# pmgbergen/porepy

Measured on AMD Instinct MI355X. Metric: cells/sec MPFA assemble+solve, 3D unstructured grid, higher is better.
Workload: dtype f64

## Files before the change

include/porefv.h:

```cpp
#ifndef POREFV_H
#define POREFV_H

#include <stddef.h>
#include <stdint.h>

#ifdef __cplusplus
extern "C" {
#endif

typedef struct pfv_ctx pfv_ctx;

typedef enum {
  PFV_OK = 0,
  PFV_ERR_SINGULAR = 1,
  PFV_ERR_CELL_SHAPE = 2,
  PFV_ERR_HIP = 3,
  PFV_ERR_ARGUMENT = 4,
  PFV_ERR_UNSUPPORTED = 5,
  PFV_ERR_NOT_CONVERGED = 6
} pfv_status;

enum {
  PFV_MAT_FLUX = 0,
  PFV_MAT_BOUND_FLUX = 1,
// ... 25 lines not shown
       PFV_PRECOND_AMG_NNS = 3,
       PFV_PRECOND_SWEEP = 4     };

enum {
  PFV_FLUXFN_LINEAR = 0,
  PFV_FLUXFN_COREY = 1,
  PFV_FLUXFN_TABLE = 2
};

enum {
  PFV_DISCR_REBUILD_TOPOLOGY = 1,
  PFV_DISCR_SKIP_VECTOR_SOURCE = 2
};

typedef struct {
  int32_t iterations;
  int32_t converged;
  double rel_residual;
  double solve_ms;
} pfv_solve_info;

typedef struct {
  double topology_ms;
  double symbolic_ms;
  double node_ms;
  double face_ms;
  double assemble_ms;
  double solve_ms;
  double bytes_written_outputs;
  int64_t num_nodes, num_sub_half_faces, sum_block_sq, max_block;
  double amg_setup_ms;
  double amg_operator_complexity;
  int64_t amg_levels, amg_coarsest_rows;
  double discretize_ms;
  int64_t solve_renumbered;
  double node_flops;
  int64_t node_table_doubles;
  int64_t amg_maps_reused;
  int64_t amg_level0_nnz;
  double amg_filter_theta;
  int64_t win_reused;
  int64_t amg_filter_layout;
  int64_t solve_launches;
  int64_t amg_setup_launches;
  int64_t node_redo;
  int64_t symbolic_reused;
  int64_t amg_stale_rematches;
  int64_t mpsa_contrast_regions;
  double mpsa_max_contrast;
  int64_t assemble_positions_kept;
  int64_t pipeline_runs;
  int64_t amg_nns_modes;
  double face_flux_ms;
  double upwind_ms;
  double transport_assemble_ms;
  double transport_advance_ms;
  int64_t transport_iterations;
  int64_t transport_gmres_retries;
  double advdiff_assemble_ms;
  double advdiff_advance_ms;
  int64_t advdiff_iterations;
  int64_t advdiff_precond_fallbacks;
  int64_t advdiff_gmres_retries;
  int64_t sweep_levels;
  int64_t sweep_core_cells;
  int64_t sweep_launches;
  double sweep_order_ms;
  int64_t sweep_direct_steps;
  int64_t sweep_direct_fallbacks;
  int64_t transport_multi_components;
  int64_t transport_multi_direct_steps;
  int64_t transport_multi_fallback_components;
  double transport_nl_ms;
  int64_t transport_nl_steps;
  int64_t transport_nl_core_iterations;
  int64_t transport_nl_components;
  double transport_react_ms;
  int64_t transport_react_steps;
  int64_t transport_react_core_iterations;
  int64_t transport_react_components;
  double transport_adjoint_ms;
  int64_t transport_adjoint_steps;
  int64_t transport_adjoint_core_iterations;
} pfv_stats;

pfv_status pfv_create(int device, pfv_ctx** out);
void pfv_destroy(pfv_ctx* h);
const char* pfv_last_error(pfv_ctx* h);
int pfv_is_device_build(void);

pfv_status pfv_set_grid(pfv_ctx* h, int nd, int64_t nc, int64_t nf, int64_t nn,
                        const double* nodes, const int32_t* cf_indptr,
                        const int32_t* cf_indices, const int8_t* cf_sign,
                        const int32_t* fn_indptr, const int32_t* fn_indices,
                        const double* face_normals, const double* face_centers,
                        const double* cell_centers, const double* face_areas);

pfv_status pfv_mpfa_set_params(pfv_ctx* h, const double* perm_33n, const uint8_t* bc_flags,
                               const double* robin_weight, double eta,
                               const double* eta_subface);

pfv_status pfv_mpfa_set_permeability(pfv_ctx* h, const double* perm_33n);

#define PFV_AD_WANT_FLUX_JACOBIAN 1u
pfv_status pfv_mpfa_ad_flux_system(pfv_ctx* h, const double* p, const double* dk_dp, const double* bc_values,
                                   const double* vector_source, const double* source, double* flux_out,
                                   uint32_t flags);

pfv_status pfv_mpfa_set_subface_bc(pfv_ctx* h, const uint8_t* bc_flags_sub, const double* robin_weight_sub);

pfv_status pfv_mpfa_discretize(pfv_ctx* h, uint32_t flags);

pfv_status pfv_tpfa_discretize(pfv_ctx* h, int vector_source_dim);

pfv_status pfv_tpfa_transmissibility_ad(pfv_ctx* h, const double* perm_33n, double* t_face, double* dt_dk);

pfv_status pfv_mpfa_discretize_faces(pfv_ctx* h, uint32_t flags, int64_t n_faces,
                                     const int32_t* faces, int keep_other_rows);

pfv_status pfv_matrix_info(pfv_ctx* h, int which, int64_t* nrows, int64_t* ncols,
                           int64_t* nnz);
pfv_status pfv_get_matrix(pfv_ctx* h, int which, int32_t* indptr, int32_t* indices,
                          double* data);
pfv_status pfv_device_memory(pfv_ctx* h, int64_t* free_bytes, int64_t* total_bytes);
pfv_status pfv_host_alloc(size_t bytes, void** out);
void pfv_host_free(void* p);
pfv_status pfv_active_size(pfv_ctx* h, int64_t* n);
pfv_status pfv_get_matrix_rows(pfv_ctx* h, int which, int64_t n_rows, const int32_t* rows, int32_t* out_indptr,
                               int32_t* out_indices, double* out_data);

pfv_status pfv_mpfa_assemble(pfv_ctx* h, const double* bc_values, const double* vector_source,
                             const double* source);
pfv_status pfv_get_rhs(pfv_ctx* h, double* b);

pfv_status pfv_spmv(pfv_ctx* h, int which, const double* x, double* y);

enum {
  PFV_BIOT_SCALAR_GRADIENT = 0,
  PFV_BIOT_DISPLACEMENT_DIVERGENCE = 1,
  PFV_BIOT_BOUNDARY_DISPLACEMENT_DIVERGENCE = 2,
  PFV_BIOT_CONSISTENCY = 3,
  PFV_BIOT_BOUND_DISPLACEMENT_PRESSURE = 4,
  PFV_BIOT_NUM_TERMS = 5
};
pfv_status pfv_biot_set_alphas(pfv_ctx* h, int nalpha, const double* alpha_k33n);
pfv_status pfv_biot_discretize_faces(pfv_ctx* h, uint32_t flags, int64_t n_faces, const int32_t* faces,
                                     int64_t n_cells, const int32_t* cells, int keep_other_rows);

pfv_status pfv_biot_discretize(pfv_ctx* h, uint32_t flags);
pfv_status pfv_biot_matrix_info(pfv_ctx* h, int term, int64_t* nrows, int64_t* ncols, int64_t* nnz);
pfv_status pfv_biot_get_matrix(pfv_ctx* h, int term, int key, int32_t* indptr, int32_t* indices,
                               double* data);

pfv_status pfv_set_system(pfv_ctx* h, int64_t n, const int32_t* indptr, const int32_t* indices,
                          const double* data, const double* rhs);

pfv_status pfv_set_periodic(pfv_ctx* h, const int32_t* native_cell, const double* shift);

pfv_status pfv_set_vectors_on_device(pfv_ctx* h, int on);

pfv_status pfv_set_preconditioner(pfv_ctx* h, int kind);

pfv_status pfv_sweep_info(pfv_ctx* h, int64_t info[4], int32_t* level, int32_t* order);

pfv_status pfv_set_near_null_space(pfv_ctx* h, int bs, int k, const double* B);

// ... 144 lines not shown
```

porepy_amd/_lib.py:

```python
from __future__ import annotations

import ctypes as C
import os

import numpy as np

_HERE = os.path.dirname(os.path.abspath(__file__))
DEFAULT_LIBRARY = os.path.join(_HERE, "csrc", "libporefv_hip.so")

MAT_FLUX, MAT_BOUND_FLUX, MAT_BOUND_PRESSURE_CELL, MAT_BOUND_PRESSURE_FACE = 0, 1, 2, 3
MAT_VECTOR_SOURCE, MAT_BOUND_PRESSURE_VECTOR_SOURCE, MAT_SYSTEM = 4, 5, 6
MAT_STRESS, MAT_BOUND_STRESS, MAT_BOUND_DISPLACEMENT_CELL, MAT_BOUND_DISPLACEMENT_FACE, MAT_MECH_SYSTEM = 7, 8, 9, 10, 11
MAT_USER_SYSTEM = 12
MAT_FLUX_JACOBIAN = 13
MAT_UPWIND, MAT_UPWIND_RHS_DIR, MAT_UPWIND_RHS_NEU, MAT_TRANSPORT_SYSTEM = 14, 15, 16, 17
MAT_ADVDIFF_SYSTEM = 18
BC_DIR, BC_NEU, BC_ROB, BC_INTERNAL = 1, 2, 4, 8
SOLVE_CG, SOLVE_BICGSTAB, SOLVE_GMRES = 0, 1, 2
PRECOND_JACOBI, PRECOND_AMG, PRECOND_BLOCK, PRECOND_AMG_NNS, PRECOND_SWEEP = 0, 1, 2, 3, 4
FLUXFN_LINEAR, FLUXFN_COREY, FLUXFN_TABLE = 0, 1, 2
DISCR_REBUILD_TOPOLOGY, DISCR_SKIP_VECTOR_SOURCE = 1, 2

STATUS_NAMES = {
    0: "ok", 1: "singular local system", 2: "unsupported cell shape", 3: "HIP error",
    4: "bad argument", 5: "unsupported size/feature", 6: "not converged",
}

EXPORTS = [
    "pfv_create", "pfv_destroy", "pfv_last_error", "pfv_is_device_build", "pfv_set_grid",
    "pfv_mpfa_set_params", "pfv_mpfa_discretize", "pfv_matrix_info", "pfv_get_matrix",
    "pfv_mpfa_assemble", "pfv_get_rhs", "pfv_spmv", "pfv_solve", "pfv_spmv_device",
    "pfv_get_device_rhs", "pfv_sync", "pfv_get_stats", "pfv_time_kernel", "pfv_debug_copy",
    "pfv_spmv_device_rows", "pfv_copy_device_vector", "pfv_set_stream",
    "pfv_mpsa_set_params", "pfv_mpsa_discretize", "pfv_mpsa_assemble",
    "pfv_mpfa_discretize_faces", "pfv_set_system", "pfv_tpfa_discretize", "pfv_mpsa_discretize_faces", "pfv_set_preconditioner", "pfv_amg_setup", "pfv_amg_setup_sharded", "pfv_amg_apply_device", "pfv_csr_from_host", "pfv_csr_from_matrix", "pfv_csr_block_diag", "pfv_csr_matmul", "pfv_csr_axpby", "pfv_csr_transpose", "pfv_csr_bmat", "pfv_csr_scale", "pfv_csr_divide", "pfv_csr_spmv", "pfv_csr_spmv_device", "pfv_csr_info", "pfv_csr_get", "pfv_csr_set_system", "pfv_csr_free", "pfv_reset_stream", "pfv_mpsa_set_robin", "pfv_mpsa_set_basis", "pfv_mpfa_set_subface_bc", "pfv_mpsa_set_subface_bc", "pfv_mpsa_set_subface_basis",
    "pfv_biot_set_alphas", "pfv_biot_discretize", "pfv_biot_matrix_info", "pfv_biot_get_matrix",
    "pfv_set_vectors_on_device", "pfv_set_periodic", "pfv_biot_discretize_faces", "pfv_solve_sharded", "pfv_tpfa_transmissibility_ad",
    "pfv_get_matrix_rows", "pfv_active_size", "pfv_device_memory",
    "pfv_rccl_unique_id", "pfv_rccl_comm_create", "pfv_rccl_set_halo_plan", "pfv_rccl_hooks", "pfv_rccl_stats",
    "pfv_rccl_last_error", "pfv_rccl_comm_destroy", "pfv_mpfa_ad_flux_system", "pfv_host_alloc", "pfv_host_free",
    "pfv_mpsa_set_subface_eta", "pfv_mpsa_set_reconstruction_eta", "pfv_mpsa_set_reconstruction_eta_subface", "pfv_get_stats_n", "pfv_set_block_preconditioner",
    "pfv_mpfa_set_permeability", "pfv_set_near_null_space", "pfv_amg_nns_level", "pfv_amg_level",
    "pfv_mpfa_face_flux", "pfv_upwind_set_bc", "pfv_upwind_discretize", "pfv_upwind_assemble", "pfv_transport_advance",
    "pfv_advdiff_assemble", "pfv_advdiff_advance", "pfv_advdiff_face_flux", "pfv_resident_flux",
    "pfv_sweep_info", "pfv_transport_advance_multi", "pfv_transport_advance_nl", "pfv_transport_advance_nl_multi",
    "pfv_transport_advance_react", "pfv_transport_adjoint_multi",
]


class SolveInfo(C.Structure):
    _fields_ = [("iterations", C.c_int32), ("converged", C.c_int32),
                ("rel_residual", C.c_double), ("solve_ms", C.c_double)]


class Stats(C.Structure):
    _fields_ = [("topology_ms", C.c_double), ("symbolic_ms", C.c_double), ("node_ms", C.c_double),
                ("face_ms", C.c_double), ("assemble_ms", C.c_double), ("solve_ms", C.c_double),
                ("bytes_written_outputs", C.c_double), ("num_nodes", C.c_int64),
                ("num_sub_half_faces", C.c_int64), ("sum_block_sq", C.c_int64),
                ("max_block", C.c_int64), ("amg_setup_ms", C.c_double),
                ("amg_operator_complexity", C.c_double), ("amg_levels", C.c_int64),
                ("amg_coarsest_rows", C.c_int64), ("discretize_ms", C.c_double), ("solve_renumbered", C.c_int64),
                ("node_flops", C.c_double), ("node_table_doubles", C.c_int64),
                ("amg_maps_reused", C.c_int64), ("amg_level0_nnz", C.c_int64), ("amg_filter_theta", C.c_double),
                ("win_reused", C.c_int64), ("amg_filter_layout", C.c_int64),
                ("solve_launches", C.c_int64), ("amg_setup_launches", C.c_int64), ("node_redo", C.c_int64),
                ("symbolic_reused", C.c_int64), ("amg_stale_rematches", C.c_int64),
                ("mpsa_contrast_regions", C.c_int64), ("mpsa_max_contrast", C.c_double), ("assemble_positions_kept", C.c_int64),
                ("pipeline_runs", C.c_int64), ("amg_nns_modes", C.c_int64),
                ("face_flux_ms", C.c_double), ("upwind_ms", C.c_double), ("transport_assemble_ms", C.c_double),
                ("transport_advance_ms", C.c_double), ("transport_iterations", C.c_int64),
                ("transport_gmres_retries", C.c_int64),
                ("advdiff_assemble_ms", C.c_double), ("advdiff_advance_ms", C.c_double),
                ("advdiff_iterations", C.c_int64), ("advdiff_precond_fallbacks", C.c_int64),
                ("advdiff_gmres_retries", C.c_int64),
                ("sweep_levels", C.c_int64), ("sweep_core_cells", C.c_int64), ("sweep_launches", C.c_int64),
                ("sweep_order_ms", C.c_double), ("sweep_direct_steps", C.c_int64),
                ("sweep_direct_fallbacks", C.c_int64),
                ("transport_multi_components", C.c_int64), ("transport_multi_direct_steps", C.c_int64),
                ("transport_multi_fallback_components", C.c_int64),
                ("transport_nl_ms", C.c_double), ("transport_nl_steps", C.c_int64),
                ("transport_nl_core_iterations", C.c_int64), ("transport_nl_components", C.c_int64),
                ("transport_react_ms", C.c_double), ("transport_react_steps", C.c_int64),
                ("transport_react_core_iterations", C.c_int64), ("transport_react_components", C.c_int64),
                ("transport_adjoint_ms", C.c_double), ("transport_adjoint_steps", C.c_int64),
                ("transport_adjoint_core_iterations", C.c_int64)]

    def as_dict(self):
        return {n: getattr(self, n) for n, _ in self._fields_}


HALO_FN = C.CFUNCTYPE(C.c_int, C.c_void_p, C.c_void_p, C.c_void_p)
ALLREDUCE_FN = C.CFUNCTYPE(C.c_int, C.c_void_p, C.c_void_p, C.c_int, C.c_void_p)


SENDRECV_FN = C.CFUNCTYPE(C.c_int, C.c_void_p, C.c_int, C.POINTER(C.c_int32), C.c_void_p, C.POINTER(C.c_int64),
                          C.c_void_p, C.POINTER(C.c_int64), C.c_void_p)
ALLGATHER_FN = C.CFUNCTYPE(C.c_int, C.c_void_p, C.c_void_p, C.c_void_p, C.c_int64, C.c_void_p)


class ShardHooks(C.Structure):
    _fields_ = [("exchange_halo", HALO_FN), ("allreduce_sum", ALLREDUCE_FN), ("user", C.c_void_p),
                ("sendrecv", SENDRECV_FN), ("allgather", ALLGATHER_FN)]


class PorefvError(RuntimeError):
    def __init__(self, status: int, message: str):
        super().__init__(f"porefv status {status} ({STATUS_NAMES.get(status, '?')}): {message}")
        self.status = status
        self.message = message


_dp = C.POINTER(C.c_double)
_ip = C.POINTER(C.c_int32)
_bp = C.POINTER(C.c_int8)
_up = C.POINTER(C.c_uint8)
_lp = C.POINTER(C.c_int64)
_h = C.c_void_p


def _bind(lib: C.CDLL) -> C.CDLL:
    lib.pfv_create.argtypes = [C.c_int, C.POINTER(_h)]
    lib.pfv_create.restype = C.c_int
    lib.pfv_destroy.argtypes = [_h]
    lib.pfv_destroy.restype = None
    lib.pfv_last_error.argtypes = [_h]
    lib.pfv_last_error.restype = C.c_char_p
    lib.pfv_is_device_build.argtypes = []
    lib.pfv_is_device_build.restype = C.c_int
    lib.pfv_set_grid.argtypes = [_h, C.c_int, C.c_int64, C.c_int64, C.c_int64, _dp, _ip, _ip, _bp,
                                 _ip, _ip, _dp, _dp, _dp, _dp]
    lib.pfv_set_grid.restype = C.c_int
    lib.pfv_mpfa_set_params.argtypes = [_h, _dp, _up, _dp, C.c_double, _dp]
    lib.pfv_mpfa_set_params.restype = C.c_int
    lib.pfv_mpfa_set_permeability.argtypes = [_h, _dp]
    lib.pfv_mpfa_set_permeability.restype = C.c_int
    lib.pfv_mpfa_discretize.argtypes = [_h, C.c_uint32]
    lib.pfv_mpfa_discretize.restype = C.c_int
    lib.pfv_mpfa_discretize_faces.argtypes = [_h, C.c_uint32, C.c_int64, _ip, C.c_int]
    lib.pfv_mpfa_discretize_faces.restype = C.c_int
    lib.pfv_mpsa_discretize_faces.argtypes = [_h, C.c_uint32, C.c_int64, _ip, C.c_int]
    lib.pfv_mpsa_discretize_faces.restype = C.c_int
    lib.pfv_biot_set_alphas.argtypes = [_h, C.c_int, _dp]
    lib.pfv_biot_set_alphas.restype = C.c_int
    lib.pfv_biot_discretize.argtypes = [_h, C.c_uint32]
    lib.pfv_biot_discretize.restype = C.c_int
    lib.pfv_biot_matrix_info.argtypes = [_h, C.c_int, _lp, _lp, _lp]
    lib.pfv_biot_matrix_info.restype = C.c_int
    lib.pfv_biot_get_matrix.argtypes = [_h, C.c_int, C.c_int, _ip, _ip, _dp]
    lib.pfv_biot_get_matrix.restype = C.c_int
    lib.pfv_mpfa_set_subface_bc.argtypes = [_h, _up, _dp]
    lib.pfv_mpfa_set_subface_bc.restype = C.c_int
    lib.pfv_mpsa_set_basis.argtypes = [_h, _dp]
    lib.pfv_mpsa_set_basis.restype = C.c_int
    lib.pfv_mpsa_set_subface_bc.argtypes = [_h, _up, _up, _up, _dp]
    lib.pfv_mpsa_set_subface_bc.restype = C.c_int
    lib.pfv_mpsa_set_subface_basis.argtypes = [_h, _dp]
    lib.pfv_mpsa_set_subface_basis.restype = C.c_int
    lib.pfv_mpsa_set_robin.argtypes = [_h, _up, _dp]
    lib.pfv_mpsa_set_robin.restype = C.c_int
    lib.pfv_mpsa_set_subface_eta.argtypes = [_h, _dp]
    lib.pfv_mpsa_set_subface_eta.restype = C.c_int
    lib.pfv_mpsa_set_reconstruction_eta.argtypes = [_h, C.c_int, C.c_double]
    lib.pfv_mpsa_set_reconstruction_eta.restype = C.c_int
    lib.pfv_mpsa_set_reconstruction_eta_subface.argtypes = [_h, _dp]
    lib.pfv_mpsa_set_reconstruction_eta_subface.restype = C.c_int
    lib.pfv_reset_stream.argtypes = [_h]
    lib.pfv_reset_stream.restype = C.c_int
    lib.pfv_amg_setup.argtypes = [_h, C.c_int64]
# ... 1413 lines not shown
```

porepy_amd/csrc/amg.inc:

```

namespace pfv {

constexpr int kAmgDenseMax = 1024;
constexpr int kAmgCoarseTargetDefault = 160;
constexpr int kAmgMaxLevels = 14;
constexpr int64_t kAmgWTopRows = 600000;
constexpr int kAmgFilterPermilBlock = 50;
constexpr int kAmgFilterPermil = 30;
constexpr int kAmgRounds = 4;
constexpr int kAmgPasses = 3;
constexpr int kAmgGentleCells = 400000;
constexpr int kGalEpl = 8;
constexpr int kGalMaxMembers = 16;
constexpr int64_t kAmgGatherRowsDefault = 32768;

struct AmgSwitches {
  int bs = 1;
  bool omega_auto = false;
  bool safe_rows = true;
  double omega = 0.95, alpha = 1.5;
  int omega_power_steps = 10;
  double omega_sigma = 1.8;
  int passes = kAmgPasses;
  bool passes_coarse_set = false;
  int passes_coarse_raw = -1;
  int rounds = kAmgRounds, rounds_raw = kAmgRounds;
  int strength_neg = 0;
  bool fp32 = true;
  double filter_theta = 0.0;
  int coarse_target = kAmgCoarseTargetDefault;
  bool gamma_set = false;
  int gamma_raw = 0;
  int gamma_levels = 1;
  int64_t fuse_rows = 30000;
  bool fuse_cycle = true;
  bool restrict_lanes = true;
  bool reuse = true, reuse_dist = true, reuse_rebuilt = true;
  int reuse_dist_min_rows = 500000;
  bool members_reuse = true, sizes_reuse = true;
  bool filter_smooth = true, rowmax_reuse = true, filter_layout_reuse = true, skip_moved_digest = true;
  bool galerkin_batched = true, filter_unroll = true, dense_lds = true;
  int64_t gather_rows = kAmgGatherRowsDefault;
};

static AmgSwitches amg_read_switches(int bs) {
  auto given = [](const char* name, int& v) {
    const char* e = std::getenv(name);
    if (e) v = std::atoi(e);
    return e != nullptr;
  };
  auto on = [](const char* name, int dflt) { return env_int(name, dflt) != 0; };
  AmgSwitches w;
  w.bs = bs;
  w.safe_rows = on("PFV_AMG_SAFE_ROWS", bs == 1 ? 1 : 0);
  int omega_pct = w.safe_rows ? 95 : 80;
  w.omega_auto = !given("PFV_AMG_OMEGA_PCT", omega_pct) && on("PFV_AMG_OMEGA_AUTO", 0);
  w.omega = 0.01 * omega_pct;
  w.alpha = 0.01 * env_int("PFV_AMG_ALPHA_PCT", 150);
  w.omega_power_steps = std::max(2, std::min(30, env_int("PFV_AMG_OMEGA_POWER_STEPS", 10)));
  w.omega_sigma = 0.01 * env_int("PFV_AMG_OMEGA_RHO_PCT", 180);
  w.passes = std::max(1, std::min(6, env_int("PFV_AMG_PASSES", kAmgPasses)));
  w.passes_coarse_set = given("PFV_AMG_PASSES_COARSE", w.passes_coarse_raw);
  w.rounds_raw = env_int("PFV_AMG_ROUNDS", kAmgRounds);
  w.rounds = std::max(1, std::min(12, w.rounds_raw));
  w.strength_neg = env_int("PFV_AMG_STRENGTH_NEG", 0);
  w.fp32 = on("PFV_AMG_FP32", 1);
  w.filter_theta = 0.001 * env_int(bs == 1 ? "PFV_AMG_FILTER_PERMIL" : "PFV_AMG_FILTER_PERMIL_BLOCK",
                                   bs == 1 ? kAmgFilterPermil : kAmgFilterPermilBlock);
  w.coarse_target = std::max(1, std::min(kAmgDenseMax, env_int("PFV_AMG_COARSE_TARGET", kAmgCoarseTargetDefault)));
  w.gamma_set = given("PFV_AMG_GAMMA", w.gamma_raw);
  w.gamma_levels = env_int("PFV_AMG_GAMMA_LEVELS", 1);
  w.fuse_rows = env_int("PFV_AMG_FUSE_ROWS", 30000);
  w.fuse_cycle = on("PFV_AMG_FUSE_CYCLE", 1);
  w.restrict_lanes = on("PFV_AMG_RESTRICT_LANES", bs == 1 ? 1 : 0);
  w.reuse = on("PFV_AMG_REUSE", 1);
  w.reuse_dist = on("PFV_AMG_REUSE_DIST", 1);
  w.reuse_rebuilt = on("PFV_AMG_REUSE_REBUILT", 1);
  w.reuse_dist_min_rows = env_int("PFV_AMG_REUSE_DIST_MIN_ROWS", 500000);
  w.members_reuse = on("PFV_AMG_MEMBERS_REUSE", 1);
  w.sizes_reuse = on("PFV_AMG_SIZES_REUSE", 1);
  w.filter_smooth = on("PFV_AMG_FILTER_SMOOTH", 1);
  w.rowmax_reuse = on("PFV_AMG_ROWMAX_REUSE", 1);
  w.filter_layout_reuse = on("PFV_AMG_FILTER_LAYOUT_REUSE", 1);
  w.skip_moved_digest = on("PFV_AMG_SKIP_MOVED_DIGEST", 1);
  w.galerkin_batched = on("PFV_AMG_GALERKIN_BATCHED", 1);
  w.filter_unroll = on("PFV_AMG_FILTER_UNROLL", 1);
  w.dense_lds = on("PFV_AMG_DENSE_LDS", 1);
  w.gather_rows = std::max<int64_t>(1, env_int("PFV_AMG_GATHER_ROWS", (int)kAmgGatherRowsDefault));
  return w;
}

static int64_t amg_maps_cfg(const AmgSwitches& w) {
  return ((((int64_t)w.passes * 16 + w.rounds_raw) * 16 + w.passes_coarse_raw + 1) * 4 + w.strength_neg) * 65536 +
         w.coarse_target * 8 + w.bs + (int64_t)(1000.0 * w.filter_theta + 0.5) * (int64_t(1) << 40);
}
static int amg_maps_tag(const AmgSwitches& w) { return w.rounds_raw * 64 + w.passes_coarse_raw + 1; }

struct AmgLevel {
  int64_t n = 0;
  int64_t m = 0;
  const CsrPattern* P = nullptr;
  const double* val = nullptr;
  CsrPattern P_own;
  Buf<double> val_own;
  Buf<float> val32;
  const float* v32 = nullptr;
  WinCsr win_own;
  const WinCsr* win = nullptr;
  Buf<double> dinv;
  Buf<int32_t> agg;
  Buf<int32_t> mptr, mem;
  int64_t nc_cells = 0;
  Buf<int32_t> pmap[6];
  int64_t pmap_n[6] = {0, 0, 0, 0, 0, 0};
  int pmap_count = 0;
  Buf<int32_t> pmp[6], pme[6];
  bool members_kept = false;
  Buf<double> x, b, t;
  Buf<double> r2, x2;
  Buf<double> u;
  double omega = 0.8;
  double rho = 0.0;
};

struct AmgWork {
  Buf<int32_t> match, pick, join, lead, a1, mp, me, cap, cnt, tcol, vin;
  Buf<uint32_t> kin, kout;
  Buf<int64_t> pos, tptr, cptr;
  Buf<double> tval, dense_work;
  Buf<int32_t> piv;
  Buf<unsigned long long> csum;
  CsrPattern P[2];
  Buf<double> V[2], D[2];
};

struct AmgPlan {
  int n_peers = 0;
  std::vector<int32_t> peers;
  std::vector<int64_t> send_ptr, recv_ptr;
  std::vector<int32_t> h_send_idx, h_recv_pos;
  Buf<int32_t> send_idx, recv_pos;
  int64_t n_send = 0, n_recv = 0;
  int64_t n_own = 0, n_halo = 0;
  std::vector<int32_t> halo_peer, halo_owner_id;
};
struct Amg;
struct AmgDist {
  ~AmgDist() {
    rows0.indptr.p = nullptr;
    rows0.indices.p = nullptr;
  }
  CsrPattern rows0;
  pfv_shard_hooks hooks{};
  int rank = 0, world = 1;
  std::vector<std::unique_ptr<AmgPlan>> plan;
  size_t kgather = 0;
  Buf<double> sbuf, rbuf, gid;
  Buf<int32_t> aext, itmp, chalo;
  std::unique_ptr<Amg> glob;
  std::vector<int64_t> gn, goff;
  int64_t gN = 0, gnmax = 0;
  Buf<int64_t> gn_d, goff_d, cnt_s, cnt_r;
  Buf<double> gsend, grecv, gb, gx, gV, gval_s, gval_r;
  Buf<int32_t> glen_s, glen_r, gcol_s, gcol_r, hal_gcell;
  CsrPattern gT, gP;
  Buf<double> gTV, gD;
  Buf<int32_t> gagg, gmp, gme;
  int64_t exchanges = 0, allgathers = 0;
  int64_t global_rows0 = 0, global_rows_level = 0;
};

struct Amg {
  Amg();
  ~Amg();
  std::unique_ptr<AmgDist> dist;
  bool no_filter = false;
  int64_t finest_cells_parent = 0;
  std::vector<std::unique_ptr<AmgLevel>> lev;
  size_t nlev = 0;
  AmgWork wk;
  int bs = 1;
  AmgSwitches sw;
  int passes = kAmgPasses;
  double omega = 0.8, alpha = 1.5;
  bool omega_auto = true;
  Buf<double> pw_a, pw_b, pw_zero, pw_part;
  Buf<double> dense;
  unsigned long long filt_layout_for = 0;
  bool filt_layout_stable = false;
  CsrPattern filtP;
  Buf<double> filtV;
  double filter_theta = 0.0;
  int64_t filt_nnz = 0;
  bool filter_level0 = false;
  WinCsr filt_win;
  struct GalSizes { int64_t ncr, annz, nnz; int maxcap; };
  std::vector<GalSizes> gal_sizes;
  unsigned long long gal_for_sum = 0;
  bool gal_use = false;
  size_t gal_k = 0;
  unsigned long long filt_win_sum = 0;
  bool maps_ok = false, reused = false;
  int64_t maps_n = -1, maps_nnz = -1, maps_cfg = 0;
  unsigned long long maps_sum = 0, maps_epoch = 0;
  int maps_tag = 0;
  int iters_fresh = -1;
  int method_fresh = -1;
  double rtol_fresh = 0.0;
  int64_t stale_rematches = 0;
  void note_iterations(int iterations, double rtol, int method, bool converged) {
    if (!valid) return;
    if (!reused) {
      iters_fresh = converged ? iterations : -1;
      rtol_fresh = rtol;
      method_fresh = method;
    } else if (iters_fresh > 0 && rtol == rtol_fresh && method == method_fresh &&
               (!converged || (double)iterations > 1.3 * (double)iters_fresh + 1.0)) {
      maps_ok = false;
      ++stale_rematches;
    }
  }
  bool dense_ok = false;
  bool restrict_lanes = true;
  bool valid = false;
  int gamma = 2, gamma_levels = 1;
  int coarse_target = 0;
  int64_t fuse_rows = 0;
  bool fuse_cycle = true;
  bool fp32 = true;
  double setup_ms = 0.0, op_complexity = 0.0;
  const CsrPattern* sysP = nullptr;
  const double* sysV = nullptr;
};

struct AmgPath {
  bool small = false;
  bool twice = false;
  bool fuse_up = false;
  bool fuse_big = false;
  bool second = false;
};
static AmgPath amg_level_path(const Amg& amg, size_t l) {
  AmgPath p;
  if (l + 1 >= amg.nlev) return p;
  const AmgLevel& L = *amg.lev[l];
  p.small = L.n <= amg.fuse_rows && !(L.win && L.win->ok);
  p.twice = amg.gamma == 2 && l >= 1 && (int)l <= amg.gamma_levels;
  p.fuse_up = p.small && l >= 1 && !p.twice;
  p.fuse_big = amg.fuse_cycle && !p.small && l >= 1;
  p.second = amg.gamma == 2 && (int)l < amg.gamma_levels && l + 2 < amg.nlev;
  return p;
}

inline Amg::Amg() = default;
inline Amg::~Amg() = default;
static bool amg_gal_cached(Amg* amg, int64_t ncr, int64_t annz, int* maxcap, int64_t* nnz) {
  if (!amg || !amg->gal_use || amg->gal_k >= amg->gal_sizes.size()) return false;
  const Amg::GalSizes& g = amg->gal_sizes[amg->gal_k];
  if (g.ncr != ncr || g.annz != annz) {
    amg->gal_use = false;
    amg->gal_sizes.resize(amg->gal_k);
    return false;
  }
  *maxcap = g.maxcap;
  *nnz = g.nnz;
  ++amg->gal_k;
  return true;
}
static void amg_gal_record(Amg* amg, int64_t ncr, int64_t annz, int maxcap, int64_t nnz) {
  if (!amg) return;
  if (amg->gal_k < amg->gal_sizes.size()) amg->gal_sizes.resize(amg->gal_k);
  amg->gal_sizes.push_back(Amg::GalSizes{ncr, annz, nnz, maxcap});
  amg->gal_k = amg->gal_sizes.size();
}

struct AmgGraph {
  const int32_t* ip;
  const int32_t* ix;
  const double* val;
  int bs;
  int neg_only;
  PFV_HD int nblk(int64_t i) const { return (ip[i * bs + 1] - ip[i * bs]) / bs; }
  PFV_HD int col(int64_t i, int k) const { return ix[ip[i * bs] + k * bs] / bs; }
  PFV_HD double w(int64_t i, int k) const {
    double s = 0.0;
    for (int a = 0; a < bs; ++a) {
      const double v = val[ip[i * bs + a] + k * bs + a];
      s += neg_only ? (v < 0.0 ? -v : 0.0) : fabs(v);
    }
    return s;
  }
};

PFV_HD inline uint32_t amg_edge_hash(int64_t i, int64_t j) {
  uint64_t a = (uint64_t)(i < j ? i : j), b = (uint64_t)(i < j ? j : i);
  uint64_t z = a * 0x9E3779B97F4A7C15ull + b + 0x7F4A7C15ull;
  z = (z ^ (z >> 30)) * 0xBF58476D1CE4E5B9ull;
  z = (z ^ (z >> 27)) * 0x94D049BB133111EBull;
  return (uint32_t)(z >> 32);
}

static void amg_pick_pass(pfv_ctx_impl& c, const AmgGraph g, int64_t nb, const int32_t* match, int want_matched,
                          int32_t* out) {
  stream_t s = c.stream;
  const size_t lds_pick = 16 * (8 + 4 + 4) + 16;
  wave_for<16>(s, nb, lds_pick, PFV_LAMBDA(const WaveCtx& w) {
    const int64_t i = w.item;
    if (match[i] >= 0) {
      if (w.lane0()) out[i] = -1;
      return;
    }
    double* cw = reinterpret_cast<double*>(w.lds);
    uint32_t* ch = reinterpret_cast<uint32_t*>(cw + 16);
// ... 797 lines not shown
    L.x.ensure(L.m);
    L.b.ensure(L.n);
  }
  L.t.ensure(L.m);
  L.v32 = nullptr;
  if (amg.fp32) {
    float* v32 = L.val32.ensure(L.P->nnz);
    const double* v64 = L.val;
    parallel_for(c.stream, L.P->nnz, PFV_LAMBDA(int64_t e) { v32[e] = (float)v64[e]; });
    L.v32 = v32;
  }
  L.nc_cells = 0;
}

static int amg_coarsen_level(pfv_ctx_impl& c, Amg& amg, size_t l, bool reuse) {
  stream_t s = c.stream;
  const AmgSwitches& w = amg.sw;
  AmgWork& wk = amg.wk;
  AmgDist* D = amg.dist.get();
  const int bs = amg.bs;
  AmgLevel& L = *amg.lev[l];
  const int64_t cells = L.n / bs;
  const CsrPattern* curP = L.P;
  const double* curV = L.val;
  if (l == 0 && amg.filter_theta > 0.0 && !amg.filter_level0) {
    amg_filter(c, w, *L.P, L.val, amg.filter_theta, amg.filtP, amg.filtV, wk, bs, amg_fill_halo0(c, D, bs));
    amg.filt_nnz = amg.filtP.nnz;
    curP = &amg.filtP;
    curV = amg.filtV.p;
  }
  int32_t* aggL = L.agg.ensure(cells);
  int64_t cur_cells = cells;
  int slot = -1;
  const int64_t finest_cells = amg.finest_cells_parent > 0 ? amg.finest_cells_parent
                                                            : (D ? D->global_rows0 : amg.lev[0]->n) / bs;
  const int coarse_default = finest_cells >= kAmgGentleCells ? std::min(2, amg.passes) : amg.passes;
  const int passes_here = (l == 0 && amg.finest_cells_parent <= 0)
                              ? amg.passes
                              : std::max(1, std::min(6, w.passes_coarse_set ? w.passes_coarse_raw : coarse_default));
  if (!reuse) L.pmap_count = 0;
  if (!reuse) L.members_kept = false;
  const bool members_reuse = reuse && L.members_kept && w.members_reuse;
  for (int pass = 0; pass < (reuse ? L.pmap_count : passes_here); ++pass) {
    int64_t nagg;
    if (reuse) {
      nagg = L.pmap_n[pass];
    } else {
      nagg = amg_pairwise(c, w, wk, *curP, curV, bs, wk.a1);
      if (nagg >= cur_cells) break;
      be_d2d(L.pmap[pass].ensure(cur_cells), wk.a1.p, sizeof(int32_t) * (size_t)cur_cells, s);
      L.pmap_n[pass] = nagg;
      L.pmap_count = pass + 1;
    }
    const int32_t* a1p = L.pmap[pass].p;
    if (!members_reuse) amg_members(c, wk, a1p, cur_cells, nagg, L.pmp[pass], L.pme[pass]);
    const int nslot = slot < 0 ? 0 : 1 - slot;
    const int32_t* amap = D ? amg_dist_extend_map(c, *D, l, a1p, cur_cells, nagg) : a1p;
    amg_galerkin(c, w, wk, *curP, curV, bs, amap, L.pmp[pass], L.pme[pass], nagg, wk.P[nslot], wk.V[nslot], wk.D[nslot],
                 D ? nullptr : &amg);
    if (D) wk.P[nslot].ncols = (nagg + D->plan[l]->n_halo) * bs;
    if (members_reuse) {
    } else if (slot < 0) {
      parallel_for(s, cells, PFV_LAMBDA(int64_t i) { aggL[i] = a1p[i]; });
    } else {
      parallel_for(s, cells, PFV_LAMBDA(int64_t i) { aggL[i] = a1p[aggL[i]]; });
    }
    slot = nslot;
    curP = &wk.P[slot];
    curV = wk.V[slot].p;
    cur_cells = nagg;
    if (nagg * bs <= w.coarse_target) break;
  }
  if (D && slot < 0) {
    amg_dist_identity_level(c, amg, *D, l, *curP, curV, aggL, cells);
    slot = 0;
  }
  if (!D && (slot < 0 || cur_cells > 0.85 * cells)) return -1;
  L.nc_cells = cur_cells;
  if (!(members_reuse && L.pmap_count > 0)) amg_members(c, wk, aggL, cells, cur_cells, L.mptr, L.mem);
  L.members_kept = L.pmap_count > 0;
  return slot;
}

static void amg_setup_finish(pfv_ctx_impl& c, Amg& amg, const CsrPattern& A, double nnz_sum, unsigned long long csum,
                             unsigned long long level0_sum) {
  const AmgSwitches& w = amg.sw;
  AmgDist* D = amg.dist.get();
  AmgLevel& Lc = *amg.lev[amg.nlev - 1];
  if (D) {
    amg_build_global(c, amg, *D, Lc, *D->plan[amg.nlev - 1]);
  } else if (Lc.n <= kAmgDenseMax) {
    amg.dense_ok = amg_dense_invert(c, w, amg.wk, *Lc.P, Lc.val, amg.dense);
  }
  amg.op_complexity = nnz_sum / (double)A.nnz;
  for (size_t k = 0; k < amg.nlev; ++k) {
    amg.lev[k]->omega = amg.omega;
    amg.lev[k]->rho = 0.0;
  }
  if (w.safe_rows) {
    for (size_t k = 0; k < amg.nlev; ++k) {
      AmgLevel& Lk = *amg.lev[k];
      if (k + 1 < amg.nlev || !amg.dense_ok) amg_safeguard_rows(c, *Lk.P, Lk.val, Lk.dinv);
    }
  }
  if (amg.omega_auto && !D) amg_estimate_omegas(c, amg);
  amg.valid = true;
  if (env_int("PFV_DEBUG_AMG", 0)) {
    std::fprintf(stderr, "amg_setup: filter theta %.3f (nnz %lld -> %lld), levels:", amg.filter_theta, (long long)A.nnz,
                 (long long)amg.filt_nnz);
    for (size_t k = 0; k < amg.nlev; ++k)
      std::fprintf(stderr, " %lld/%lld(w%.3f)", (long long)amg.lev[k]->n, (long long)amg.lev[k]->P->nnz, amg.lev[k]->omega);
    std::fprintf(stderr, " reuse %d\n", (int)amg.reused);
  }
  amg.gal_for_sum = D ? 0ull : level0_sum;
  if (w.reuse && (!D || csum != 0)) {
    amg.maps_ok = true;
    amg.maps_n = A.nrows;
    amg.maps_nnz = A.nnz;
    amg.maps_cfg = amg_maps_cfg(w);
    amg.maps_sum = csum;
    amg.maps_epoch = c.symbolic_epoch;
    amg.maps_tag = amg_maps_tag(w);
  }
}

static void amg_setup(pfv_ctx_impl& c, Amg& amg, const CsrPattern& A, const double* val, int bs,
                      const double* diag, const WinCsr* win0) {
  stream_t s = c.stream;
  Timer tm;
  tm.start(s);
  AmgDist* D = amg.dist.get();
  amg.bs = bs;
  amg.valid = amg.dense_ok = false;
  amg.sysP = &A;
  amg.sysV = val;
  if (A.nrows % bs) throw Error(PFV_ERR_ARGUMENT, "AMG: system size is not a multiple of the block size");
  AmgSwitches& w = amg.sw = amg_read_switches(bs);
  if (amg.no_filter) w.filter_theta = 0.0;
  if (amg.coarse_target > 0) w.coarse_target = std::min(kAmgDenseMax, amg.coarse_target);
  amg.omega_auto = w.omega_auto;
  amg.omega = w.omega;
  amg.alpha = w.alpha;
  amg.passes = w.passes;
  amg.fp32 = w.fp32;
  amg.filter_theta = w.filter_theta;
  amg.gamma_levels = w.gamma_levels;
  amg.fuse_rows = w.fuse_rows;
  amg.fuse_cycle = w.fuse_cycle;
  amg.restrict_lanes = w.restrict_lanes;
  unsigned long long csum = 0;
  const bool reuse = amg_decide_reuse(c, amg, A, csum);
  const int64_t rows_for_shape = D ? D->global_rows0 / D->world : A.nrows;
  amg.gamma = std::max(1, std::min(2, w.gamma_set ? w.gamma_raw : (rows_for_shape >= kAmgWTopRows ? 2 : 1)));
  amg.maps_ok = false;
  amg.reused = reuse;
  if (bs > 1) amg_check_full_blocks(c, A, bs);
  unsigned long long level0_sum = amg_setup_level0(c, amg, A, val, diag, win0, csum);
  amg.gal_use = reuse && !D && level0_sum != 0 && amg.gal_for_sum == level0_sum && w.sizes_reuse;
  amg.gal_k = 0;
  if (!amg.gal_use) amg.gal_sizes.clear();
  double nnz_sum = 0.0;
  size_t l = 0;
  while (true) {
    AmgLevel& L = amg_level(amg, l);
    nnz_sum += (double)L.P->nnz;
    amg_level_buffers(c, amg, L, l);
    if (D ? (l >= 1 && l == D->kgather) : (L.n <= w.coarse_target || (int)l + 1 >= kAmgMaxLevels)) break;
    const int slot = amg_coarsen_level(c, amg, l, reuse);
    if (slot < 0) break;
    AmgLevel& Ln = amg_level(amg, l + 1);
    Ln.n = L.nc_cells * bs;
    amg_swap_pattern(Ln.P_own, amg.wk.P[slot]);
    Ln.val_own.swap(amg.wk.V[slot]);
    Ln.dinv.swap(amg.wk.D[slot]);
    Ln.P = &Ln.P_own;
    Ln.val = Ln.val_own.p;
    Ln.win = nullptr;
    Ln.m = Ln.n;
    if (D) {
      amg_dist_rename_halo(c, *D, l, L.agg, L.nc_cells, bs, Ln);
      amg_dist_decide_gather(c, *D, l, Ln.n, w.gather_rows);
    }
    if (Ln.n > w.coarse_target && Ln.P_own.nnz >= 200000) {
      win_build(c, Ln.P_own, Ln.win_own);
      Ln.win = &Ln.win_own;
    }
    ++l;
  }
  amg.nlev = l + 1;
  amg_setup_finish(c, amg, A, nnz_sum, csum, level0_sum);
  amg.setup_ms = tm.stop(s);
}


#ifndef PFV_EMULATE
template <int L, int U, class VT, int MODE>
__global__ void __launch_bounds__(256) k_amg_spmv(int64_t nrows, const int32_t* __restrict__ indptr,
                                                  const int32_t* __restrict__ indices,
                                                  const VT* __restrict__ val, const double* __restrict__ x,
                                                  double* __restrict__ y, const double* __restrict__ b,
                                                  const double* __restrict__ dinv, double omega, const SpmvFuse F) {
  const int lane = threadIdx.x % L;
  const int64_t row = (int64_t)blockIdx.x * (256 / L) + threadIdx.x / L;
  if (row >= nrows) return;
  const int a = indptr[row], e = indptr[row + 1];
  double sum = 0.0;
  for (int p = a + lane; p < e; p += L * U) {
    int col[U];
    double v[U];
#pragma unroll
    for (int u = 0; u < U; ++u) {
      const int pp = p + u * L;
      const bool ok = pp < e;
      const int pc = ok ? pp : a;
      col[u] = indices[pc];
      const double vv = (double)val[pc];
      v[u] = ok ? vv : 0.0;
    }
#pragma unroll
    for (int u = 0; u < U; ++u) sum += v[u] * (MODE == 4 ? spmv_prolonged(F, x, col[u]) : x[col[u]]);
  }
#pragma unroll
  for (int o = L / 2; o > 0; o >>= 1) sum += __shfl_down(sum, o, L);
  if (lane == 0) {
    if (MODE == 1) y[row] = x[row] + omega * dinv[row] * (b[row] - sum);
    else if (MODE == 4) y[row] = spmv_prolonged(F, x, row) + omega * dinv[row] * (b[row] - sum);
    else if (MODE == 5) {
      const double res = b[row] - sum;
      y[row] = res;
      F.y2[row] = omega * dinv[row] * res;
    } else y[row] = sum;
  }
}
template <int L, class VT, int MODE>
static void launch_amg_spmv(stream_t s, int U, int64_t nrows, const int32_t* ip, const int32_t* ix, const VT* val,
                            const double* x, double* y, const double* b, const double* dinv, double omega,
                            const SpmvFuse& F) {
  const unsigned blocks = (unsigned)((nrows + 256 / L - 1) / (256 / L));
  if (U <= 2)
    PFV_LAUNCH(HIP_KERNEL_NAME(k_amg_spmv<L, 2, VT, MODE>), dim3(blocks), dim3(256), 0, s, nrows, ip, ix,
                       val, x, y, b, dinv, omega, F);
  else if (U <= 4)
    PFV_LAUNCH(HIP_KERNEL_NAME(k_amg_spmv<L, 4, VT, MODE>), dim3(blocks), dim3(256), 0, s, nrows, ip, ix,
                       val, x, y, b, dinv, omega, F);
  else
    PFV_LAUNCH(HIP_KERNEL_NAME(k_amg_spmv<L, 6, VT, MODE>), dim3(blocks), dim3(256), 0, s, nrows, ip, ix,
                       val, x, y, b, dinv, omega, F);
}
#endif

template <class VT, int MODE>
static void amg_spmv_t(pfv_ctx_impl& c, const CsrPattern& P, const VT* val, const double* x, double* y,
                       const double* b, const double* dinv, double omega, const SpmvFuse& F = SpmvFuse{}) {
  stream_t s = c.stream;
  const int64_t nrows = P.nrows;
  if (nrows == 0) return;
  const int32_t* ip = P.indptr;
  const int32_t* ix = P.indices;
#ifdef PFV_EMULATE
  parallel_for(s, nrows, PFV_LAMBDA(int64_t r) {
    double sum = 0.0;
    for (int p = ip[r]; p < ip[r + 1]; ++p) sum += (double)val[p] * (MODE == 4 ? spmv_prolonged(F, x, ix[p]) : x[ix[p]]);
    if (MODE == 1) y[r] = x[r] + omega * dinv[r] * (b[r] - sum);
    else if (MODE == 4) y[r] = spmv_prolonged(F, x, r) + omega * dinv[r] * (b[r] - sum);
    else if (MODE == 5) {
      const double res = b[r] - sum;
      y[r] = res;
      F.y2[r] = omega * dinv[r] * res;
    } else y[r] = sum;
  });
#else
  const double avg = (double)P.nnz / (double)nrows;
  const int L = avg <= 20 ? 8 : (avg <= 160 ? 16 : 32);
// ... 240 lines not shown
        for (int j = 0; j < w.width; ++j) sum += sh[j];
        bc[R] = sum;
        if (next_smooths) xn[R] = omega_n * dn[R] * sum;
      }
      w.lsync();
    });
  }
}

static double* amg_cycle(pfv_ctx_impl& c, Amg& amg, size_t l, const double* b, double* x, bool x_is_presmoothed,
                         int visit) {
  stream_t s = c.stream;
  AmgLevel& L = *amg.lev[l];
  const int64_t n = L.n;
  const double omega = L.omega, alpha = amg.alpha;
  const double* dinv = L.dinv;
  double* t = L.t;
  if (l + 1 == amg.nlev) {
    if (amg.dense_ok) {
      amg_dense_apply(c, amg.dense, n, b, x);
    } else {
      parallel_for(s, n, PFV_LAMBDA(int64_t i) { x[i] = omega * dinv[i] * b[i]; });
      for (int sweep = 0; sweep < 2; ++sweep) {
        amg_spmv(c, amg, L, x, t, b);
        amg_spmv(c, amg, L, t, x, b);
      }
    }
    return x;
  }
  AmgLevel& Ln = *amg.lev[l + 1];
  const int bs = amg.bs;
  const double omega_n = Ln.omega;
  const AmgPath path = amg_level_path(amg, l);
  const bool small = path.small;
  const bool twice = path.twice;
  const bool fuse_up = path.fuse_up;
  const bool fuse_big = path.fuse_big;
  if (!x_is_presmoothed) parallel_for(s, n, PFV_LAMBDA(int64_t i) { x[i] = omega * dinv[i] * b[i]; });
  const bool next_smooths = l + 2 < amg.nlev;
  if (small) {
    if (L.v32) amg_restrict_residual<float>(c, amg, L, Ln, L.v32, b, x, next_smooths);
    else amg_restrict_residual<double>(c, amg, L, Ln, L.val, b, x, next_smooths);
  } else {
    amg_spmv(c, amg, L, x, t, nullptr);
    amg_restrict(c, amg, L, Ln, b, t, next_smooths);
  }
  double* xc = amg_cycle(c, amg, l + 1, Ln.b, Ln.x, next_smooths, 0);
  const double* xc2 = nullptr;
  if (path.second) {
    double* r2 = Ln.r2.ensure(Ln.n);
    double* x2 = Ln.x2.ensure(Ln.n);
    const double* bcn = Ln.b;
    const double* x2r;
    if (amg.fuse_cycle) {
      SpmvFuse F;
      F.y2 = x2;
      amg_spmv_fused<5>(c, Ln, xc, r2, bcn, F);
      x2r = amg_cycle(c, amg, l + 1, r2, x2, true, 1);
    } else {
      double* tn = Ln.t;
      amg_spmv(c, amg, Ln, xc, tn, nullptr);
      parallel_for(s, Ln.n, PFV_LAMBDA(int64_t i) { r2[i] = bcn[i] - tn[i]; });
      x2r = amg_cycle(c, amg, l + 1, r2, x2, false, 1);
    }
    if (amg.fuse_cycle && !fuse_up) xc2 = x2r;
    else parallel_for(s, Ln.n, PFV_LAMBDA(int64_t i) { xc[i] += x2r[i]; });
  }
  if (fuse_up) {
    if (L.v32) amg_prolong_smooth<float>(c, amg, L, L.v32, b, x, xc, t);
    else amg_prolong_smooth<double>(c, amg, L, L.val, b, x, xc, t);
    return t;
  }
  if (fuse_big) {
    double* out = (twice && visit == 0) ? L.u.ensure(n) : t;
    SpmvFuse F;
    F.xc = xc;
    F.xc2 = xc2;
    F.agg = L.agg;
    F.bs = bs;
    F.alpha = alpha;
    amg_spmv_fused<4>(c, L, x, out, b, F);
    return out;
  }
  {
    const int32_t* agg = L.agg;
    parallel_for(s, n, PFV_LAMBDA(int64_t r) {
      const int64_t i = r / bs;
      const int64_t a = (int64_t)agg[i] * bs + (r - i * bs);
      t[r] = x[r] + alpha * (xc2 ? xc[a] + xc2[a] : xc[a]);
    });
  }
  amg_spmv(c, amg, L, t, x, b);
  return x;
}

struct BlockPc {
  struct Blk {
    int64_t p0 = 0, p1 = 0;
    CsrPattern P;
    Buf<double> val, diag;
    std::unique_ptr<Amg> amg;
  };
  std::vector<int64_t> ptr;
  std::vector<std::unique_ptr<Blk>> blk;
  bool gs = true;
  const double* for_val = nullptr;
  Buf<double> tmp;
  double setup_ms = 0.0;
};

static void blockpc_extract(pfv_ctx_impl& c, const CsrPattern& P, const double* val, BlockPc::Blk& B) {
  stream_t s = c.stream;
  const int64_t p0 = B.p0, n = B.p1 - B.p0;
  const int32_t* ip = P.indptr;
  const int32_t* ix = P.indices;
  Buf<int32_t> len;
  Buf<int64_t> pos;
  int32_t* ln = len.ensure(n + 1);
  int64_t* ps = pos.ensure(n + 1);
  const int64_t p1 = B.p1;
  parallel_for(s, n, PFV_LAMBDA(int64_t r) {
    int m = 0;
    for (int e = ip[p0 + r]; e < ip[p0 + r + 1]; ++e) m += (ix[e] >= p0 && ix[e] < p1) ? 1 : 0;
    ln[r] = m;
  });
  exclusive_scan<int32_t, int64_t>(s, c.scratch, ln, ps, (size_t)n);
  const int64_t nnz = read_scalar<int64_t>(s, ps + n);
  if (nnz >= (int64_t(1) << 31)) throw Error(PFV_ERR_UNSUPPORTED, "block with more than 2^31 entries");
  B.P.nrows = B.P.ncols = n;
  B.P.nnz = nnz;
  int32_t* bip = B.P.indptr.ensure(n + 1);
  int32_t* bix = B.P.indices.ensure(std::max<int64_t>(nnz, 1));
  double* bv = B.val.ensure(std::max<int64_t>(nnz, 1));
  double* bd = B.diag.ensure(n);
  int32_t* st = c.status.ensure(16);
  be_memset(st + 11, 0, sizeof(int32_t), s);
  parallel_for(s, n + 1, PFV_LAMBDA(int64_t r) { bip[r] = (int32_t)ps[r]; });
  parallel_for(s, n, PFV_LAMBDA(int64_t r) {
    int64_t o = ps[r];
    double d = 0.0;
    for (int e = ip[p0 + r]; e < ip[p0 + r + 1]; ++e) {
      const int cc = ix[e];
      if (cc >= p0 && cc < p1) {
        bix[o] = (int32_t)(cc - p0);
        bv[o] = val[e];
        if (cc == p0 + r) d = val[e];
        ++o;
      }
    }
    bd[r] = d;
    if (!(d != 0.0)) atomic_max_i32(st + 11, 1);
  });
  if (read_scalar<int32_t>(s, st + 11))
    throw Error(PFV_ERR_ARGUMENT, "block preconditioner: a diagonal entry is zero (permute the rows first: "
                                  "porepy_amd.solvers.match_rows)");
  B.P.max_row = 0;
}

static void blockpc_setup(pfv_ctx_impl& c, BlockPc& M, const CsrPattern& P, const double* val) {
  Timer tm;
  tm.start(c.stream);
  const size_t nb = M.ptr.size() - 1;
  while (M.blk.size() < nb) M.blk.push_back(std::make_unique<BlockPc::Blk>());
  M.blk.resize(nb);
  for (size_t k = 0; k < nb; ++k) {
    BlockPc::Blk& B = *M.blk[k];
// ... 72 lines not shown
```

Before: 32.56 million.

## Precompute A·P on finest AMG level to fuse post-correction smoothing

During AMG setup, builds a compressed A·P matrix for the finest level by summing each row's fp32 entries per coarse aggregate, deduplicated in LDS. In the V-cycle's upward pass on level 0, a new kernel applies the prolongated correction and one Jacobi smoothing step in one pass. It uses A·P times the coarse correction, so it no longer forms t = x + alpha·P·xc and then runs a full fine-level SpMV. This trades extra setup work and memory for a smaller, fused per-cycle operation, at the cost of double-precision values and a serial fallback for long rows.

```diff
diff --git a/include/porefv.h b/include/porefv.h
--- a/include/porefv.h
+++ b/include/porefv.h
@@ -131,6 +131,7 @@
   double transport_adjoint_ms;
   int64_t transport_adjoint_steps;
   int64_t transport_adjoint_core_iterations;
+  int64_t amg_ap_nnz;
 } pfv_stats;
 
 pfv_status pfv_create(int device, pfv_ctx** out);
diff --git a/porepy_amd/_lib.py b/porepy_amd/_lib.py
--- a/porepy_amd/_lib.py
+++ b/porepy_amd/_lib.py
@@ -84,7 +84,7 @@
                 ("transport_react_ms", C.c_double), ("transport_react_steps", C.c_int64),
                 ("transport_react_core_iterations", C.c_int64), ("transport_react_components", C.c_int64),
                 ("transport_adjoint_ms", C.c_double), ("transport_adjoint_steps", C.c_int64),
-                ("transport_adjoint_core_iterations", C.c_int64)]
+                ("transport_adjoint_core_iterations", C.c_int64), ("amg_ap_nnz", C.c_int64)]
 
     def as_dict(self):
         return {n: getattr(self, n) for n, _ in self._fields_}
diff --git a/porepy_amd/csrc/amg.inc b/porepy_amd/csrc/amg.inc
--- a/porepy_amd/csrc/amg.inc
+++ b/porepy_amd/csrc/amg.inc
@@ -41,6 +41,7 @@
   bool filter_smooth = true, rowmax_reuse = true, filter_layout_reuse = true, skip_moved_digest = true;
   bool galerkin_batched = true, filter_unroll = true, dense_lds = true;
   int64_t gather_rows = kAmgGatherRowsDefault;
+  bool post_ap = true;
 };
 
 static AmgSwitches amg_read_switches(int bs) {
@@ -87,6 +88,7 @@
   w.filter_unroll = on("PFV_AMG_FILTER_UNROLL", 1);
   w.dense_lds = on("PFV_AMG_DENSE_LDS", 1);
   w.gather_rows = std::max<int64_t>(1, env_int("PFV_AMG_GATHER_ROWS", (int)kAmgGatherRowsDefault));
+  w.post_ap = on("PFV_AMG_POST_AP", 1);
   return w;
 }
 
@@ -229,6 +231,11 @@
   bool fuse_cycle = true;
   bool fp32 = true;
   double setup_ms = 0.0, op_complexity = 0.0;
+  bool ap_ok = false;
+  int64_t ap_nnz = 0;
+  Buf<int32_t> ap_ptr, ap_col, ap_len;
+  Buf<int64_t> ap_pos;
+  Buf<double> ap_val;
   const CsrPattern* sysP = nullptr;
   const double* sysV = nullptr;
 };
@@ -1192,6 +1199,212 @@
   return slot;
 }
 
+constexpr int kApKeys = 128;
+constexpr int kApChunk = 8;
+static void amg_build_ap(pfv_ctx_impl& c, Amg& amg) {
+  stream_t s = c.stream;
+  amg.ap_ok = false;
+  amg.ap_nnz = 0;
+  AmgLevel& L = *amg.lev[0];
+  if (!amg.sw.post_ap || amg.bs != 1 || amg.dist || amg.no_filter || amg.finest_cells_parent > 0 || !L.v32 ||
+      L.nc_cells <= 0 || L.n != L.m || (L.n <= amg.fuse_rows && !(L.win && L.win->ok)))
+    return;
+  const int64_t n = L.n, fnnz = L.P->nnz;
+  int32_t *sx, *al, *cp, *cx;
+  int64_t* pos;
+  double *sv, *cv;
+  try {
+    sx = amg.wk.tcol.ensure(std::max<int64_t>(fnnz, 1));
+    sv = amg.wk.tval.ensure(std::max<int64_t>(fnnz, 1));
+    al = amg.ap_len.ensure(n + 1);
+    pos = amg.ap_pos.ensure(n + 1);
+    cp = amg.ap_ptr.ensure(n + 1);
+    cx = amg.ap_col.ensure(std::max<int64_t>(fnnz, 1));
+    cv = amg.ap_val.ensure(std::max<int64_t>(fnnz, 1));
+  } catch (const Error&) {
+#ifndef PFV_EMULATE
+    (void)hipGetLastError();
+#endif
+    amg.ap_col.release();
+    amg.ap_val.release();
+    return;
+  }
+  const int32_t* fp = L.P->indptr;
+  const int32_t* ix = L.P->indices;
+  const float* v32 = L.v32;
+  const int32_t* agg = L.agg;
+  wave_for<16>(s, n, (kApKeys + kApChunk) * (2 * sizeof(int32_t) + sizeof(float)) + 16, PFV_LAMBDA(const WaveCtx& w) {
+    const int64_t r = w.item;
+    const int p0 = fp[r], len = fp[r + 1] - p0;
+    if (len > kApKeys) {
+      if (w.lane0()) {
+        int cnt = 0;
+        for (int e = 0; e < len; ++e) {
+          const int32_t k = agg[ix[p0 + e]];
+          const double v = (double)v32[p0 + e];
+          int q = 0;
+          while (q < cnt && sx[p0 + q] < k) ++q;
+          if (q < cnt && sx[p0 + q] == k) {
+            sv[p0 + q] += v;
+          } else {
+            for (int m = cnt; m > q; --m) {
+              sx[p0 + m] = sx[p0 + m - 1];
+              sv[p0 + m] = sv[p0 + m - 1];
+            }
+            sx[p0 + q] = k;
+            sv[p0 + q] = 0.0 + v;
+            ++cnt;
+          }
+        }
+        al[r] = cnt;
+      }
+      return;
+    }
+    uint32_t* kh = reinterpret_cast<uint32_t*>(w.lds);
+    int32_t* dupf = reinterpret_cast<int32_t*>(kh + kApKeys + kApChunk);
+    float* vs = reinterpret_cast<float*>(dupf + kApKeys + kApChunk);
+    PFV_LANES(e, len) {
+      kh[e] = (uint32_t)agg[ix[p0 + e]];
+      vs[e] = v32[p0 + e];
+    }
+    PFV_LANES(u, kApChunk) kh[len + u] = 0xffffffffu;
+    w.lsync();
+    PFV_LANES(e, len) {
+      const uint32_t k = kh[e];
+      int dup = 0;
+      for (int q0 = 0; q0 < e; q0 += kApChunk) {
+#pragma unroll
+        for (int u = 0; u < kApChunk; ++u) dup |= (q0 + u < e && kh[q0 + u] == k) ? 1 : 0;
+      }
+      dupf[e] = dup;
+    }
+    w.lsync();
+    PFV_LANES(e, len) kh[e] |= dupf[e] ? 0x80000000u : 0u;
+    w.lsync();
+    PFV_LANES(e, len) {
+      const uint32_t ke = kh[e];
+      const uint32_t k = ke & 0x7fffffffu;
+      int rank = 0, cnt = 0;
+      double sum = 0.0;
+      for (int q0 = 0; q0 < len; q0 += kApChunk) {
+#pragma unroll
+        for (int u = 0; u < kApChunk; ++u) {
+          const uint32_t kq = kh[q0 + u];
+          const float vq = vs[q0 + u];
+          rank += kq < k ? 1 : 0;
+          cnt += (int)((kq >> 31) ^ 1u);
+          if ((kq & 0x7fffffffu) == k) sum += (double)vq;
+        }
+      }
+      if (ke == k) {
+        sx[p0 + rank] = (int32_t)k;
+        sv[p0 + rank] = sum;
+      }
+      if (e == 0) al[r] = cnt;
+    }
+    if (len == 0 && w.lane0()) al[r] = 0;
+    w.lsync();
+  });
+  exclusive_scan<int32_t, int64_t>(s, c.scratch, al, pos, (size_t)n);
+  wave_for<8>(s, n, 16, PFV_LAMBDA(const WaveCtx& w) {
+    const int64_t r = w.item;
+    const int p0 = fp[r];
+    const int64_t o = pos[r];
+    PFV_LANES(q, al[r]) {
+      cx[o + q] = sx[p0 + q];
+      cv[o + q] = sv[p0 + q];
+    }
+    if (w.lane0()) {
+      cp[r] = (int32_t)o;
+      if (r + 1 == n) cp[n] = (int32_t)pos[n];
+    }
+  });
+  amg.ap_ok = true;
+}
+
+#ifndef PFV_EMULATE
+template <int CH>
+__global__ void __launch_bounds__(256) k_amg_post_ap(int64_t nrows, const int32_t* __restrict__ ap,
+                                                     const int32_t* __restrict__ ax, const double* __restrict__ av,
+                                                     const int32_t* __restrict__ agg, const double* __restrict__ xc,
+                                                     const double* __restrict__ xc2, const double* __restrict__ t,
+                                                     const double* __restrict__ b, const double* __restrict__ dinv,
+                                                     double omega, double alpha, double* x) {
+  __shared__ double prod[CH];
+  const int64_t row0 = (int64_t)blockIdx.x * 256;
+  const int64_t row1 = row0 + 256 < nrows ? row0 + 256 : nrows;
+  const int64_t row = row0 + threadIdx.x;
+  const bool live = row < nrows;
+  const int a0 = ap[row0], e0 = ap[row1];
+  int a = 0, e = 0;
+  double x0 = 0.0, tr = 0.0, br = 0.0, dr = 0.0, xr = 0.0;
+  if (live) {
+    a = ap[row];
+    e = ap[row + 1];
+    const int k = agg[row];
+    x0 = x[row];
+    tr = t[row];
+    br = b[row];
+    dr = dinv[row];
+    xr = xc[k];
+    if (xc2) xr += xc2[k];
+  }
+  double sum = 0.0;
+  for (int c0 = a0; c0 < e0; c0 += CH) {
+    constexpr int U = CH / 256;
+    int k[U];
+    double v[U], xs[U];
+#pragma unroll
+    for (int u = 0; u < U; ++u) {
+      const int p = c0 + u * 256 + (int)threadIdx.x;
+      const bool ok = p < e0;
+      k[u] = ok ? ax[p] : -1;
+      v[u] = ok ? av[p] : 0.0;
+    }
+#pragma unroll
+    for (int u = 0; u < U; ++u) {
+      xs[u] = k[u] >= 0 ? xc[k[u]] : 0.0;
+      if (xc2 && k[u] >= 0) xs[u] += xc2[k[u]];
+    }
+#pragma unroll
+    for (int u = 0; u < U; ++u) prod[u * 256 + threadIdx.x] = v[u] * xs[u];
+    __syncthreads();
+    const int lo = a > c0 ? a : c0, hi = e < c0 + CH ? e : c0 + CH;
+    for (int p = lo; p < hi; ++p) sum += prod[p - c0];
+    __syncthreads();
+  }
+  if (live) {
+    const double tt = x0 + alpha * xr;
+    x[row] = tt + omega * dr * (br - (tr + alpha * sum));
+  }
+}
+#endif
+static void amg_post_ap(pfv_ctx_impl& c, const Amg& amg, const AmgLevel& L, const double* b, const double* t,
+                        const double* xc, const double* xc2, double* x) {
+  stream_t s = c.stream;
+  const int64_t n = L.n;
+  const int32_t* ap = amg.ap_ptr;
+  const int32_t* ax = amg.ap_col;
+  const double* av = amg.ap_val;
+  const int32_t* agg = L.agg;
+  const double* dinv = L.dinv;
+  const double omega = L.omega, alpha = amg.alpha;
+#ifdef PFV_EMULATE
+  parallel_for(s, n, PFV_LAMBDA(int64_t r) {
+    double sum = 0.0;
+    for (int p = ap[r]; p < ap[r + 1]; ++p) sum += av[p] * (xc2 ? xc[ax[p]] + xc2[ax[p]] : xc[ax[p]]);
+    const int k = agg[r];
+    const double tt = x[r] + alpha * (xc2 ? xc[k] + xc2[k] : xc[k]);
+    x[r] = tt + omega * dinv[r] * (b[r] - (t[r] + alpha * sum));
+  });
+#else
+  const unsigned blocks = (unsigned)((n + 255) / 256);
+  PFV_LAUNCH(HIP_KERNEL_NAME(k_amg_post_ap<2048>), dim3(blocks), dim3(256), 0, s, n, ap, ax, av, agg, xc, xc2, t, b, dinv,
+             omega, alpha, x);
+  PFV_HIP_CHECK(hipGetLastError());
+#endif
+}
+
 static void amg_setup_finish(pfv_ctx_impl& c, Amg& amg, const CsrPattern& A, double nnz_sum, unsigned long long csum,
                              unsigned long long level0_sum) {
   const AmgSwitches& w = amg.sw;
@@ -1241,7 +1454,8 @@
   tm.start(s);
   AmgDist* D = amg.dist.get();
   amg.bs = bs;
-  amg.valid = amg.dense_ok = false;
+  amg.valid = amg.dense_ok = amg.ap_ok = false;
+  amg.ap_nnz = 0;
   amg.sysP = &A;
   amg.sysV = val;
   if (A.nrows % bs) throw Error(PFV_ERR_ARGUMENT, "AMG: system size is not a multiple of the block size");
@@ -1278,6 +1492,7 @@
     if (D ? (l >= 1 && l == D->kgather) : (L.n <= w.coarse_target || (int)l + 1 >= kAmgMaxLevels)) break;
     const int slot = amg_coarsen_level(c, amg, l, reuse);
     if (slot < 0) break;
+    if (l == 0) amg_build_ap(c, amg);
     AmgLevel& Ln = amg_level(amg, l + 1);
     Ln.n = L.nc_cells * bs;
     amg_swap_pattern(Ln.P_own, amg.wk.P[slot]);
@@ -1299,6 +1514,8 @@
   }
   amg.nlev = l + 1;
   amg_setup_finish(c, amg, A, nnz_sum, csum, level0_sum);
+  if (amg.ap_ok) amg.ap_nnz = read_scalar<int64_t>(s, amg.ap_pos.p + amg.lev[0]->n);
+  c.stats.amg_ap_nnz = amg.ap_nnz;
   amg.setup_ms = tm.stop(s);
 }
 
@@ -1705,6 +1922,10 @@
     amg_spmv_fused<4>(c, L, x, out, b, F);
     return out;
   }
+  if (l == 0 && amg.ap_ok && !small) {
+    amg_post_ap(c, amg, L, b, t, xc, xc2, x);
+    return x;
+  }
   {
     const int32_t* agg = L.agg;
     parallel_for(s, n, PFV_LAMBDA(int64_t r) {
```

Result: faster. 33.24 million (median of 6 runs) (+2.1%).
